# CUHK-AIM-Group/Depth-Aware-Endoscopy-SR

Hardware: AMD Instinct MI355X
Metric: LR frames/sec fwd+bwd at x8 (128x160 LR) (higher is better)
Workload: dtype f32; 1 GPU; Kvasir x8 synthetic, batch=16 per GPU, fp32, DepthNet nb=16 nf=64 L=256 K=10 (BASELINE.json configs[1]); step = fwd + L1 + dynamic loss + bwd + Adam; global_batch=16, scale=8, parallelism=dp1, mode=train, device=cuda, full=False, hip_graph=False

## Files before the change

depth-aware-endoscopy-sr_amd/csrc/edge.hip:

```cpp
#include "dasr_common.h"
#include "bf16.h"

extern "C" int dasr_version(void) { return 100; }
extern "C" int dasr_is_device_build(void) { return DASR_DEVICE_BUILD; }
extern "C" const char* dasr_error_string(int code) {
    switch (code) {
        case DASR_OK: return "ok";
        case DASR_E_NULL: return "null pointer argument";
        case DASR_E_SHAPE: return "inconsistent or non-positive sizes";
        case DASR_E_UNSUPPORTED: return "unsupported configuration";
        case DASR_E_WORKSPACE: return "workspace too small";
        default: return code > 0 ? "hip runtime error (hipError_t)" : "unknown error";
    }
}

__global__ void k_nchw_to_nhwc(const float* __restrict__ src, float* __restrict__ dst, int C, int HW, size_t n) {
    for (size_t i = (size_t)blockIdx.x * blockDim.x + threadIdx.x; i < n; i += (size_t)gridDim.x * blockDim.x) {
        size_t c = i % C, p = (i / C) % HW, b = i / ((size_t)C * HW);
        dst[i] = src[(b * C + c) * HW + p];
    }
}
__global__ void k_nhwc_to_nchw(const float* __restrict__ src, float* __restrict__ dst, int C, int HW, size_t n) {
    for (size_t i = (size_t)blockIdx.x * blockDim.x + threadIdx.x; i < n; i += (size_t)gridDim.x * blockDim.x) {
        size_t p = i % HW, c = (i / HW) % C, b = i / ((size_t)C * HW);
// ... 12 lines not shown
    DASR_CHECK_SHAPE(B > 0 && C > 0 && H > 0 && W > 0);
    size_t n = (size_t)B * C * H * W;
    DASR_LAUNCH(k_nhwc_to_nchw, dim3(dasr_ew_grid(n)), dim3(256), 0, stream, src, dst, C, H * W, n);
    DASR_RETURN_LAUNCH_STATUS();
}

__global__ void k_clamp_to_nchw(const float* __restrict__ y, float* __restrict__ out, int C, int HW, size_t n, float lo,
                                float hi) {
    for (size_t i = (size_t)blockIdx.x * blockDim.x + threadIdx.x; i < n; i += (size_t)gridDim.x * blockDim.x) {
        size_t p = i % HW, c = (i / HW) % C, b = i / ((size_t)C * HW);
        float v = y[(b * HW + p) * C + c];
        out[i] = fminf(fmaxf(v, lo), hi);
    }
}
__global__ void k_clamp_to_nchw_bwd(const float* __restrict__ dout, const float* __restrict__ y, float* __restrict__ dy,
                                    int C, int HW, size_t n, float lo, float hi) {
    for (size_t i = (size_t)blockIdx.x * blockDim.x + threadIdx.x; i < n; i += (size_t)gridDim.x * blockDim.x) {
        size_t c = i % C, p = (i / C) % HW, b = i / ((size_t)C * HW);
        float v = y[i];
        float g = dout[(b * C + c) * HW + p];
        dy[i] = (v >= lo && v <= hi) ? g : 0.f;
    }
}
extern "C" int dasr_clamp_to_nchw(const float* y, float* out, int B, int C, int H, int W, float lo, float hi,
                                  void* stream) {
    DASR_CHECK_PTR(y); DASR_CHECK_PTR(out);
    DASR_CHECK_SHAPE(B > 0 && C > 0 && H > 0 && W > 0);
    size_t n = (size_t)B * C * H * W;
    DASR_LAUNCH(k_clamp_to_nchw, dim3(dasr_ew_grid(n)), dim3(256), 0, stream, y, out, C, H * W, n, lo, hi);
    DASR_RETURN_LAUNCH_STATUS();
}
extern "C" int dasr_clamp_to_nchw_bwd(const float* dout, const float* y, float* dy, int B, int C, int H, int W, float lo,
                                      float hi, void* stream) {
    DASR_CHECK_PTR(dout); DASR_CHECK_PTR(y); DASR_CHECK_PTR(dy);
    DASR_CHECK_SHAPE(B > 0 && C > 0 && H > 0 && W > 0);
    size_t n = (size_t)B * C * H * W;
    DASR_LAUNCH(k_clamp_to_nchw_bwd, dim3(dasr_ew_grid(n)), dim3(256), 0, stream, dout, y, dy, C, H * W, n, lo, hi);
    DASR_RETURN_LAUNCH_STATUS();
}

__global__ void k_resize_nearest(const float* __restrict__ src, float* __restrict__ dst, int h, int w, int H, int W,
                                 size_t n) {
    float sh = (float)h / (float)H, sw = (float)w / (float)W;
    for (size_t i = (size_t)blockIdx.x * blockDim.x + threadIdx.x; i < n; i += (size_t)gridDim.x * blockDim.x) {
        int X = (int)(i % W), Y = (int)((i / W) % H);
        size_t bc = i / ((size_t)W * H);
        int y = (int)floorf((float)Y * sh); if (y > h - 1) y = h - 1;
        int x = (int)floorf((float)X * sw); if (x > w - 1) x = w - 1;
        dst[i] = src[(bc * h + y) * w + x];
    }
}
extern "C" int dasr_resize_nearest_nchw(const float* src, float* dst, int BC, int h, int w, int H, int W, void* stream) {
    DASR_CHECK_PTR(src); DASR_CHECK_PTR(dst);
    DASR_CHECK_SHAPE(BC > 0 && h > 0 && w > 0 && H > 0 && W > 0);
    size_t n = (size_t)BC * H * W;
    DASR_LAUNCH(k_resize_nearest, dim3(dasr_ew_grid(n)), dim3(256), 0, stream, src, dst, h, w, H, W, n);
    DASR_RETURN_LAUNCH_STATUS();
}

__global__ void k_resize_nearest_u8(const unsigned char* __restrict__ src, unsigned char* __restrict__ dst, int h, int w,
// ... 92 lines not shown
```

depth-aware-endoscopy-sr_amd/csrc/loss.hip:

```cpp
#include <stdint.h>

#include "dasr_common.h"

#define LOSS_MAXK 16

__global__ void __launch_bounds__(256) k_loss_sums(const float* __restrict__ sr, const float* __restrict__ hr,
                                                   const unsigned char* __restrict__ region, float* __restrict__ sums,
                                                   int B, int C, int h, int w, int s, int K) {
    __shared__ float red[2 * LOSS_MAXK + 2];
    for (int i = threadIdx.x; i < 2 * K + 1; i += 256) red[i] = 0.f;
    __syncthreads();
    const int W = w * s, H = h * s;
    const size_t nruns = (size_t)B * C * H * w;
    float l1 = 0.f;
    for (size_t r = (size_t)blockIdx.x * 256 + threadIdx.x; r < nruns; r += (size_t)gridDim.x * 256) {
        const int lx = (int)(r % w);
        const int Y = (int)((r / w) % H);
        const size_t bc = r / ((size_t)w * H);
        const int b = (int)(bc / C);
        const int k = region[((size_t)b * h + Y / s) * w + lx];
        const float* ps = sr + (bc * H + Y) * W + (size_t)lx * s;
        const float* ph = hr + (bc * H + Y) * W + (size_t)lx * s;
        float num = 0.f;
        for (int j = 0; j < s; ++j) {
            const float d = ps[j] - ph[j], ad = fabsf(d);
            l1 += ad;
            num += ad < 1.f ? 0.5f * d * d : ad - 0.5f;
        }
        if (k < K) {
            atomicAdd(&red[k], num);
            atomicAdd(&red[K + k], (float)s);
        }
    }
    for (int off = 32; off > 0; off >>= 1) l1 += __shfl_down(l1, off, 64);
    if ((threadIdx.x & 63) == 0) atomicAdd(&red[2 * K], l1);
    __syncthreads();
    for (int i = threadIdx.x; i < 2 * K + 1; i += 256) atomicAdd(&sums[i], red[i]);
}

__global__ void __launch_bounds__(256) k_loss_bwd(const float* __restrict__ sr, const float* __restrict__ hr,
                                                  const unsigned char* __restrict__ region,
                                                  const float* __restrict__ dsums, float* __restrict__ dsr, int B,
                                                  int C, int h, int w, int s, int K) {
    const int W = w * s, H = h * s;
    const size_t n = (size_t)B * C * H * W;
    const float dl1 = dsums[2 * K];
    for (size_t i = (size_t)blockIdx.x * 256 + threadIdx.x; i < n; i += (size_t)gridDim.x * 256) {
        const int X = (int)(i % W), Y = (int)((i / W) % H);
        const int b = (int)(i / ((size_t)W * H * C));
        const int k = region[((size_t)b * h + Y / s) * w + X / s];
        const float d = sr[i] - hr[i];
        const float sg = d > 0.f ? 1.f : (d < 0.f ? -1.f : 0.f);
        float g = dl1 * sg;
        if (k < K) g += dsums[k] * (fabsf(d) < 1.f ? d : sg);
        dsr[i] = g;
    }
}

extern "C" int dasr_loss_sums(const float* sr, const float* hr, const unsigned char* region, float* sums, int B, int C,
                              int h, int w, int scale, int K, void* stream) {
    DASR_CHECK_PTR(sr); DASR_CHECK_PTR(hr); DASR_CHECK_PTR(region); DASR_CHECK_PTR(sums);
    DASR_CHECK_SHAPE(B > 0 && C > 0 && h > 0 && w > 0 && scale > 0 && K > 0);
    if (K > LOSS_MAXK) return DASR_E_UNSUPPORTED;
    hipError_t e = hipMemsetAsync(sums, 0, sizeof(float) * (2 * K + 1), (hipStream_t)stream);
    if (e != hipSuccess) return (int)e;
    size_t nruns = (size_t)B * C * h * scale * w;
    DASR_LAUNCH(k_loss_sums, dim3(dasr_ew_grid(nruns)), dim3(256), 0, stream, sr, hr, region, sums, B, C, h, w, scale, K);
    DASR_RETURN_LAUNCH_STATUS();
}

extern "C" int dasr_loss_bwd(const float* sr, const float* hr, const unsigned char* region, const float* dsums,
                             float* dsr, int B, int C, int h, int w, int scale, int K, void* stream) {
    DASR_CHECK_PTR(sr); DASR_CHECK_PTR(hr); DASR_CHECK_PTR(region); DASR_CHECK_PTR(dsums); DASR_CHECK_PTR(dsr);
    DASR_CHECK_SHAPE(B > 0 && C > 0 && h > 0 && w > 0 && scale > 0 && K > 0);
    if (K > LOSS_MAXK) return DASR_E_UNSUPPORTED;
    size_t n = (size_t)B * C * h * scale * w * scale;
    DASR_LAUNCH(k_loss_bwd, dim3(dasr_ew_grid(n)), dim3(256), 0, stream, sr, hr, region, dsums, dsr, B, C, h, w, scale, K);
    DASR_RETURN_LAUNCH_STATUS();
}

__device__ __forceinline__ float loss_sign(float v) { return v > 0.f ? 1.f : (v < 0.f ? -1.f : 0.f); }

template <int K>
__device__ __forceinline__ void loss_soft_px(float d, const float (&m)[K], float (&num)[K], float& l1) {
    l1 += fabsf(d);
#pragma unroll
    for (int k = 0; k < K; ++k) {
        const float u = m[k] * d, au = fabsf(u);
        num[k] += au < 1.f ? 0.5f * u * u : au - 0.5f;
    }
// ... 89 lines not shown
    const float dl1 = dsums[2 * K];
    for (size_t r = (size_t)blockIdx.x * 256 + threadIdx.x; r < nruns; r += (size_t)gridDim.x * 256) {
        bool first_row;
        const size_t off = loss_soft_run<K>(r, mask, C, h, w, s, m, first_row);
#pragma unroll
        for (int k = 0; k < K; ++k) coef[k] = dnum[k] * m[k];
        for (int c = 0; c < C; ++c) {
            const float* ps = sr + off + c * plane;
            const float* ph = hr + off + c * plane;
            float* pd = dsr + off + c * plane;
            if (VEC) {
                for (int j = 0; j < s; j += 4) {
                    const f32x4 d = *reinterpret_cast<const f32x4*>(ps + j) - *reinterpret_cast<const f32x4*>(ph + j);
                    f32x4 g;
#pragma unroll
                    for (int i = 0; i < 4; ++i) g[i] = loss_soft_px_bwd<K>(d[i], dl1, m, coef);
                    *reinterpret_cast<f32x4*>(pd + j) = g;
                }
            } else {
                for (int j = 0; j < s; ++j) pd[j] = loss_soft_px_bwd<K>(ps[j] - ph[j], dl1, m, coef);
            }
        }
    }
}

static inline bool loss_aligned16(const void* a, const void* b, const void* c = nullptr) {
    return (((uintptr_t)a | (uintptr_t)b | (uintptr_t)c) & 15) == 0;
}

#define LOSS_SOFT_CASE(KK, KERNEL, ...)                                                                  \
    case KK:                                                                                             \
        if (vec) DASR_LAUNCH((KERNEL<KK, true>), dim3(dasr_ew_grid(nruns)), dim3(256), 0, stream, __VA_ARGS__);  \
        else DASR_LAUNCH((KERNEL<KK, false>), dim3(dasr_ew_grid(nruns)), dim3(256), 0, stream, __VA_ARGS__);     \
        break;
#define LOSS_SOFT_DISPATCH(KERNEL, ...)                                                                          \
    switch (K) {                                                                                                 \
        LOSS_SOFT_CASE(1, KERNEL, __VA_ARGS__) LOSS_SOFT_CASE(2, KERNEL, __VA_ARGS__) LOSS_SOFT_CASE(3, KERNEL, __VA_ARGS__)    \
        LOSS_SOFT_CASE(4, KERNEL, __VA_ARGS__) LOSS_SOFT_CASE(5, KERNEL, __VA_ARGS__) LOSS_SOFT_CASE(6, KERNEL, __VA_ARGS__)    \
        LOSS_SOFT_CASE(7, KERNEL, __VA_ARGS__) LOSS_SOFT_CASE(8, KERNEL, __VA_ARGS__) LOSS_SOFT_CASE(9, KERNEL, __VA_ARGS__)    \
        LOSS_SOFT_CASE(10, KERNEL, __VA_ARGS__) LOSS_SOFT_CASE(11, KERNEL, __VA_ARGS__) LOSS_SOFT_CASE(12, KERNEL, __VA_ARGS__) \
        LOSS_SOFT_CASE(13, KERNEL, __VA_ARGS__) LOSS_SOFT_CASE(14, KERNEL, __VA_ARGS__) LOSS_SOFT_CASE(15, KERNEL, __VA_ARGS__) \
        LOSS_SOFT_CASE(16, KERNEL, __VA_ARGS__)                                                                  \
        default: return DASR_E_UNSUPPORTED;                                                                      \
    }

extern "C" int dasr_loss_sums_soft(const float* sr, const float* hr, const float* mask, float* sums, int B, int C, int h,
                                   int w, int scale, int K, void* stream) {
    DASR_CHECK_PTR(sr); DASR_CHECK_PTR(hr); DASR_CHECK_PTR(mask); DASR_CHECK_PTR(sums);
    DASR_CHECK_SHAPE(B > 0 && C > 0 && h > 0 && w > 0 && scale > 0 && K > 0);
    if (K > LOSS_MAXK) return DASR_E_UNSUPPORTED;
// ... 316 lines not shown
```

depth-aware-endoscopy-sr_amd/depthnet.py:

```python
import contextlib
import math

import torch
import torch.nn as nn

from . import graph
from .tape import Tape, Var


def _default_conv_init_(weight, bias, fan_in):
    bound = 1.0 / math.sqrt(fan_in)
    with torch.no_grad():
        weight.uniform_(-bound, bound)
        if bias is not None:
            bias.uniform_(-bound, bound)


class _PlainConv(nn.Module):

    def __init__(self, cin, cout, k):
        super().__init__()
        self.cin, self.cout, self.k = cin, cout, k
        self.weight = nn.Parameter(torch.empty(cout, cin, k, k))
        self.bias = nn.Parameter(torch.empty(cout))
# ... 64 lines not shown

    forward = _PlainConv.forward


class _Encoder(nn.Module):

    def __init__(self, in_nc, latent):
        super().__init__()
        self.layer1 = _WNConv(in_nc, 32)
        self.layer2 = _WNConv(32, 64)
        self.layer3 = _WNConv(64, 128)
        self.layer4 = _WNConv(128, latent, transposed=True)
        self.layer5 = _WNConv(latent, latent)

    forward = _PlainConv.forward


def _device_guard(t):
    return torch.cuda.device(t.device) if t.is_cuda else contextlib.nullcontext()


class _DepthNetFunction(torch.autograd.Function):
    @staticmethod
    def forward(ctx, net, act_dtype, inp, depth_map, depth_mask, region, *params):
        tape = Tape(enabled=True, act_dtype=act_dtype)
        tape.prepack = net._prepack_for(inp.device, act_dtype)
        pvars = [Var(p.detach(), p.requires_grad, name) for name, p in zip(net._param_names, params)]
        P = {v.name: v for v in pvars}
        out = graph.depthnet_forward(tape, P, net.cfg, net._consts(inp.device), inp.detach().contiguous(),
                                     depth_map.detach().contiguous(), depth_mask.detach().contiguous(), region)
        ctx.tape, ctx.pvars, ctx.out = tape, pvars, out
        ctx.hook = getattr(net, "_grad_bucket_hook", None)
        return out.data

    @staticmethod
    def backward(ctx, dout):
        tape, pvars, out = ctx.tape, ctx.pvars, ctx.out
        if tape is None:
            raise RuntimeError("DepthNet: backward called twice on the same forward")
        out.grad = dout.contiguous()
        if ctx.hook is not None:
            hook = ctx.hook
            tape.on_mark = lambda: hook(pvars)
        with _device_guard(dout):
            tape.backward()
        grads = tuple(v.grad for v in pvars)
        for v in pvars:
            v.grad = None
        ctx.tape = ctx.pvars = ctx.out = ctx.hook = None
        return (None, None, None, None, None, None) + grads


class DepthNet(nn.Module):
    def __init__(self, which_ResBlk_depth=[], in_nc=3, out_nc=3, nf=64, nb=16, scale=4, input_para=10, min=0.0,
                 max=1.0, depth_latent_ch=256, depthRangeNum=10, norm_type='weight_norm', use_trainable_params=True,
                 norm_gamma=0.1, norm_beta=0.1, ablate_depth_matrix=False, ablate_depth_block=False):
        super().__init__()
        if norm_type != 'weight_norm':
            raise NotImplementedError("dasr_amd.DepthNet: only norm_type='weight_norm' (all shipped ymls) is built")
        if ablate_depth_matrix or ablate_depth_block:
            raise NotImplementedError("dasr_amd.DepthNet: the ablate_* variants are outside the hot path (SURVEY §8b)")
        if scale not in (2, 3, 4, 8):
            raise NotImplementedError("dasr_amd.DepthNet: scale must be 2, 3, 4 or 8")
        self.scale, self.min, self.max, self.para = scale, min, max, input_para
        self.num_blocks = nb
        self.which_ResBlk_depth = list(which_ResBlk_depth)
        self.isBaseline = len(self.which_ResBlk_depth) == 0
        self.ablate_depth_matrix, self.ablate_depth_block = False, False
        self.cfg = dict(which_ResBlk_depth=self.which_ResBlk_depth, in_nc=in_nc, out_nc=out_nc, nf=nf, nb=nb,
                        scale=scale, depth_latent_ch=depth_latent_ch, depthRangeNum=depthRangeNum,
                        use_trainable_params=use_trainable_params, norm_gamma=norm_gamma, norm_beta=norm_beta,
                        out_min=float(min), out_max=float(max))

# ... 80 lines not shown
            P = {name: Var(p.detach(), False, name) for name, p in zip(self._param_names, params)}
            return graph.depthnet_infer_nhwc(tape, P, self.cfg, self._consts(x_nhwc.device), x_nhwc, depthMap, depthMask,
                                             graph.attached_region(depthMask))

    def forward(self, input, depthMap, depthMask):
        with _device_guard(input):
            return self._forward(input, depthMap, depthMask)

    def _forward(self, input, depthMap, depthMask):
        params = self._resolve_params()
        for t, nm in ((depthMap, "depthMap"), (depthMask, "depthMask")):
            if t.device != input.device:
                raise ValueError("DepthNet: %s is on %s, input on %s" % (nm, t.device, input.device))
        if params and params[0].device != input.device:
            raise ValueError("DepthNet: parameters on %s, input on %s" % (params[0].device, input.device))
        for t, nm in ((input, "input"), (depthMap, "depthMap"), (depthMask, "depthMask")):
            if t.dtype != torch.float32:
                raise TypeError("DepthNet: %s must be float32" % nm)
        if input.dim() != 4 or depthMap.dim() != 4 or depthMask.dim() != 4:
            raise ValueError("DepthNet: expected 4-D NCHW tensors")
        region = graph.attached_region(depthMask)
        act_dtype = self._act_dtype(input.device)
        if torch.is_grad_enabled() and any(p.requires_grad for p in params):
            return _DepthNetFunction.apply(self, act_dtype, input, depthMap, depthMask, region, *params)
        tape = Tape(enabled=False, act_dtype=act_dtype)
        if not self.training:
            if not hasattr(self, "_fold_cache"):
                object.__setattr__(self, "_fold_cache", {})
            tape.fold_cache = self._fold_cache
        P = {name: Var(p.detach(), False, name) for name, p in zip(self._param_names, params)}
        out = graph.depthnet_forward(tape, P, self.cfg, self._consts(input.device), input.detach().contiguous(),
                                     depthMap.detach().contiguous(), depthMask.detach().contiguous(), region)
        return out.data
```

depth-aware-endoscopy-sr_amd/graph.py:

```python
import math

import torch

from . import ops
from .tape import Tape, Var, accum


FUSE_DGRAD_ACT = False
FUSE_C9_DGRAD_ACT = True
FUSE_SPLIT_DGRAD_ACT = True

SIDE_STREAM = True
import os as _os
import threading as _threading
TAIL_WGRAD_SIDE = False
FUSE_INSTNORM_STATS = False
ENCODER_S2D = True
SPLIT_BF16 = True
SPLIT_WGRAD = True
SPLIT_PIECES = 2
FUSE_AMAX = True
SPLIT_CONV9 = True
SPLIT_MIN_PIXELS = 1 << 14
WGRAD_STREAM = False
_SIDE = {}
_SIDE_LOCK = _threading.Lock()


def _side_stream(device, which="branch"):
    key = (str(device), which)
    with _SIDE_LOCK:
        if key not in _SIDE:
            _SIDE[key] = torch.cuda.Stream(device=device, priority=-1)
# ... 720 lines not shown
    s2d_ok = all(P["encoder.layer%d.weight_v" % i].data.shape[0] % 32 == 0 and
                 P["encoder.layer%d.weight_v" % i].data.shape[1] % 32 == 0 for i in (2, 3, 4, 5))
    if len(cfg["which_ResBlk_depth"]) > 0 and tape.act_dtype == torch.bfloat16 and ENCODER_S2D and s2d_ok:
        def s2(name, x, act, valid_hw=None):
            return conv(tape, space_to_depth2(tape, x, valid_hw), expand_s2(tape, _wn(tape, P, name)), P[name + ".bias"],
                        act=act)
        e2 = s2("encoder.layer2", e1, L)
        e3 = s2("encoder.layer3", e2, L)
        w4, b4 = expand_t2(tape, _wn(tape, P, "encoder.layer4", True), P["encoder.layer4.bias"])
        e4 = conv(tape, e3, w4, b4, act=L, ps_r=2)
        H3, W3 = e3.data.shape[1], e3.data.shape[2]
        e5 = to_f32(tape, s2("encoder.layer5", e4, ops.ACT_NONE, (2 * H3 - 1, 2 * W3 - 1)))
        st = region_pool(tape, e5, depth_mask)
    elif len(cfg["which_ResBlk_depth"]) > 0:
        e2 = conv(tape, e1, _wn(tape, P, "encoder.layer2"), P["encoder.layer2.bias"], stride=2, act=L)
        e3 = conv(tape, e2, _wn(tape, P, "encoder.layer3"), P["encoder.layer3.bias"], stride=2, act=L)
        e4 = conv(tape, e3, _wn(tape, P, "encoder.layer4", True), P["encoder.layer4.bias"], stride=2,
                  transposed=True, act=L)
        e5 = conv(tape, e4, _wn(tape, P, "encoder.layer5"), P["encoder.layer5.bias"], stride=2)
        st = region_pool(tape, e5, depth_mask)
    return e1, e5, st


def depthnet_forward(tape, P, cfg, consts, inp, depth_map, depth_mask, region=None):
    pp = tape.prepack
    if pp is not None and not (PREPACK and tape.enabled and pp.lock.acquire(blocking=False)):
        pp = tape.prepack = None
    try:
        if pp is not None:
            pp.begin(P, Prepack.signature(inp, tape.act_dtype))
        out = _depthnet_forward(tape, P, cfg, consts, inp, depth_map, depth_mask, region)
        if pp is not None:
            pp.finish()
        return out
    finally:
        if pp is not None:
            pp.lock.release()


def depthnet_infer_nhwc(tape, P, cfg, consts, x_nhwc, depth_map, depth_mask, region=None):
    if tape.enabled:
        raise ValueError("depthnet_infer_nhwc is an inference entry: the tape must be off")
    return _depthnet_forward(tape, P, cfg, consts, x_nhwc, depth_map, depth_mask, region, nhwc=True).data


def _depthnet_forward(tape, P, cfg, consts, inp, depth_map, depth_mask, region, *, nhwc=False):
    plan = block_plan(cfg)
    nb, scale = cfg["nb"], cfg["scale"]
    B = inp.shape[0]
    x0 = Var(inp if nhwc else ops.nchw_to_nhwc(inp))
    dm = Var(depth_map.reshape(B, depth_map.shape[2], depth_map.shape[3], 1))
    L = ops.ACT_LRELU
    e1, _e5, st = encoder_forward(tape, P, cfg, x0, depth_mask)
    mask_pack = MaskPack(depth_mask, region) if st is not None else None
    adt = tape.act_dtype
    e1h = to_bf16(tape, e1) if adt == torch.bfloat16 else e1
    h1 = conv(tape, e1h, _wn(tape, P, "head.0", dtype=adt), P["head.0.bias"], act=L)
    fea_bef = conv(tape, h1, _wn(tape, P, "head.2", dtype=adt), P["head.2.bias"], act=L)

    executed = list(range(nb - 3)) + [nb - 2, nb - 1]
    branch = {}
    side = _side_stream(inp.device) if (SIDE_STREAM and inp.is_cuda and mask_pack is not None) else None
    if side is not None:
        main = torch.cuda.current_stream()
        side.wait_stream(main)
        feat_hw = {}
        hw = (x0.data.shape[1], x0.data.shape[2])
        for i in executed:
            if i == nb - 2 and scale == 8:
# ... 15 lines not shown
                branch[i] = tuple(pair)

    def run_block(i, x):
        name, kind, _ = plan[i]
        if kind == "depth":
            return depth_block(tape, P, name, x, dm, mask_pack, st, consts, branch.get(i))
        return classic_block(tape, P, name, x)

    fea = fea_bef
    tape.mark()
    for i in range(nb - 3):
        fea = run_block(i, fea)
        if i == (nb - 3) // 2 - 1:
            tape.mark()
    fea = add(tape, fea, fea_bef)
    tape.mark()
    if scale == 8:
        fea = upscale(tape, P, "upscale1", fea, 2, True)
    fea = run_block(nb - 2, fea)
    if scale >= 4:
        fea = upscale(tape, P, "upscale2", fea, 2, True)
    fea = run_block(nb - 1, fea)
    fea = upscale(tape, P, "upscale3", fea, 3 if scale == 3 else 2, False)
    y = conv(tape, fea, pack(tape, P["conv_output.weight"]), P["conv_output.bias"], pad=4, side_wgrad=True)
    if nhwc:
        return y
    lo, hi = cfg["out_min"], cfg["out_max"]
    out = Var(ops.clamp_to_nchw(y.data, lo, hi), True)

    def bwd():
        if out.grad is None:
            return
        accum(y, ops.clamp_to_nchw_bwd(out.grad, y.data, lo, hi))
        out.grad = None

    tape.record(bwd)
    return out
```

depth-aware-endoscopy-sr_amd/harness.py:

```python
import math

import torch
import torch.nn.functional as F


def cosine_restart_lr(step, base_lr=1e-3, T_period=(20000, 20000, 20000, 20000),
                      restarts=(20000, 40000, 60000), weights=(1, 1, 1), eta_min=1e-7):
    last_restart, T, w = 0, T_period[0], 1.0
    for j, r in enumerate(restarts):
        if step >= r:
            last_restart, T, w = r, T_period[j + 1], weights[j]
    return eta_min + (base_lr * w - eta_min) * (1 + math.cos(math.pi * (step - last_restart) / T)) / 2


def _world(group=None):
    if torch.distributed.is_available() and torch.distributed.is_initialized():
        return torch.distributed.get_world_size(group)
    return 1


class _RegionSums(torch.autograd.Function):

    @staticmethod
    def forward(ctx, sr, hr, region, K):
        from . import ops
        sr_c, hr_c = sr.contiguous(), hr.contiguous()
        ctx.save_for_backward(sr_c, hr_c, region)
        ctx.K = K
        return ops.loss_sums(sr_c, hr_c, region, K)

    @staticmethod
    def backward(ctx, dsums):
        from . import ops
        sr, hr, region = ctx.saved_tensors
        return ops.loss_bwd(sr, hr, region, dsums.contiguous(), ctx.K), None, None, None


class _RegionSumsSoft(torch.autograd.Function):

    @staticmethod
    def forward(ctx, sr, hr, mask, K):
        from . import ops
        sr_c, hr_c, mask_c = sr.contiguous(), hr.contiguous(), mask.detach().contiguous()
        ctx.save_for_backward(sr_c, hr_c, mask_c)
        ctx.K = K
        return ops.loss_sums_soft(sr_c, hr_c, mask_c, K)

    @staticmethod
    def backward(ctx, dsums):
        from . import ops
        sr, hr, mask = ctx.saved_tensors
        return ops.loss_bwd_soft(sr, hr, mask, dsums.contiguous(), ctx.K), None, None, None


def ssim_torch(img1, img2):
    from .validate import _window_1d
    g = _window_1d().unsqueeze(1)
# ... 601 lines not shown
```

depth-aware-endoscopy-sr_amd/ops.py:

```python
import ctypes

import torch

from . import _lib

ACT_NONE, ACT_RELU, ACT_LRELU = 0, 1, 2
IN_EPS = 1e-5


BF16 = torch.bfloat16


def _p(t, allow_none=False):
    return _lib.ptr(t, allow_none)


def _pa(t, allow_none=False):
    if t is None:
        return _lib.ptr(t, allow_none)
    return _lib.ptr(t, allow_none, dtype=t.dtype if t.dtype in (torch.float32, BF16) else torch.float32)


def _is_bf(*ts):
    kinds = {t.dtype for t in ts if t is not None}
# ... 740 lines not shown
    dfeat = torch.empty(feat_shape, dtype=torch.float32, device=dout.device)
    _call("dasr_region_pool_bwd", _p(dout), _p(maskr), _p(area), _p(dfeat), B, K, L, h, w)
    return dfeat


def loss_sums(sr, hr, region, K):
    B, C, H, W = sr.shape
    _, h, w = region.shape
    scale = H // h
    assert H == h * scale and W == w * scale
    sums = empty((2 * K + 1,), sr)
    _call("dasr_loss_sums", _p(sr), _p(hr), _lib.ptr(region, dtype=torch.uint8), _p(sums), B, C, h, w, scale, K)
    return sums


def loss_bwd(sr, hr, region, dsums, K):
    B, C, H, W = sr.shape
    _, h, w = region.shape
    dsr = torch.empty_like(sr)
    _call("dasr_loss_bwd", _p(sr), _p(hr), _lib.ptr(region, dtype=torch.uint8), _p(dsums), _p(dsr), B, C, h, w, H // h, K)
    return dsr


LOSS_MAX_REGIONS = 16


def _soft_loss_dims(sr, mask, K):
    B, C, H, W = sr.shape
    Bm, Km, h, w = mask.shape
    scale = H // h
    assert (Bm, Km) == (B, K) and H == h * scale and W == w * scale
    return B, C, h, w, scale


def loss_sums_soft(sr, hr, mask, K):
    B, C, h, w, scale = _soft_loss_dims(sr, mask, K)
    assert hr.shape == sr.shape
    sums = empty((2 * K + 1,), sr)
    _call("dasr_loss_sums_soft", _p(sr), _p(hr), _p(mask), _p(sums), B, C, h, w, scale, K)
    return sums


def loss_bwd_soft(sr, hr, mask, dsums, K):
    B, C, h, w, scale = _soft_loss_dims(sr, mask, K)
    assert hr.shape == sr.shape and dsums.numel() == 2 * K + 1
    dsr = torch.empty_like(sr)
# ... 197 lines not shown
```

include/dasr.h:

```cpp
#ifndef DASR_H
#define DASR_H

#include <stddef.h>
#include <stdint.h>

#ifdef __cplusplus
extern "C" {
#endif

#define DASR_OK 0
#define DASR_E_NULL (-1)
#define DASR_E_SHAPE (-2)
#define DASR_E_UNSUPPORTED (-3)
#define DASR_E_WORKSPACE (-4)

#define DASR_ACT_NONE 0
#define DASR_ACT_RELU 1
#define DASR_ACT_LRELU02 2

int dasr_version(void);
const char* dasr_error_string(int code);
int dasr_is_device_build(void);

int dasr_nchw_to_nhwc(const float* src, float* dst, int B, int C, int H, int W, void* stream);
// ... 117 lines not shown
                  float* dbias_gamma, float* dbias_beta, float* dalpha_gamma, float* dalpha_beta, float* dres,
                  float* dt_amax, float* dgb2_amax, void* workspace, size_t workspace_bytes, int relu, int B, int H, int W,
                  int C, int K, float eps, void* stream);

int dasr_sean_soft_mask_max_regions(void);

int dasr_region_pool_fwd(const float* feat, const float* mask, float* maskr, float* area, float* out, int B, int K,
                         int L, int h, int w, int H, int W, void* stream);
int dasr_region_pool_bwd(const float* dout, const float* maskr, const float* area, float* dfeat, int B, int K, int L,
                         int h, int w, void* stream);

size_t dasr_depth_to_masks_workspace(int B, int HW);
int dasr_depth_to_masks(const float* depth, const float* fixed_edges, float* masks, unsigned char* region,
                        void* workspace, size_t workspace_bytes, int B, int HW, int K, void* stream);

size_t dasr_depth_to_masks_soft_workspace(int B, int HW);
int dasr_depth_to_masks_soft(const float* depth, float* masks, void* workspace, size_t workspace_bytes, int B, int HW,
                             int K, float width, int fixed_range, void* stream);

int dasr_loss_sums(const float* sr, const float* hr, const unsigned char* region, float* sums, int B, int C, int h,
                   int w, int scale, int K, void* stream);
int dasr_loss_bwd(const float* sr, const float* hr, const unsigned char* region, const float* dsums, float* dsr, int B,
                  int C, int h, int w, int scale, int K, void* stream);
int dasr_loss_sums_soft(const float* sr, const float* hr, const float* mask, float* sums, int B, int C, int h, int w,
                        int scale, int K, void* stream);
int dasr_loss_bwd_soft(const float* sr, const float* hr, const float* mask, const float* dsums, float* dsr, int B, int C,
                       int h, int w, int scale, int K, void* stream);
#define DASR_CRIT_NONE (-1)
#define DASR_CRIT_L1 0
#define DASR_CRIT_L2 1
#define DASR_CRIT_CB 2
#define DASR_CRIT_SMOOTHL1 3
int dasr_loss_sums_crit(const float* sr, const float* hr, const unsigned char* region, float* sums, int B, int C, int h,
                        int w, int scale, int K, int pixel_crit, int crit_a, int crit_b, void* stream);
int dasr_loss_bwd_crit(const float* sr, const float* hr, const unsigned char* region, const float* dsums, float* dsr,
                       int B, int C, int h, int w, int scale, int K, int pixel_crit, int crit_a, int crit_b, void* stream);
int dasr_loss_sums_soft_crit(const float* sr, const float* hr, const float* mask, float* sums, int B, int C, int h, int w,
                             int scale, int K, int pixel_crit, int crit_a, int crit_b, void* stream);
int dasr_loss_bwd_soft_crit(const float* sr, const float* hr, const float* mask, const float* dsums, float* dsr, int B,
                            int C, int h, int w, int scale, int K, int pixel_crit, int crit_a, int crit_b, void* stream);

int dasr_add(const float* a, const float* b, float* out, size_t n, void* stream);
int dasr_accumulate(float* dst, const float* src, size_t n, void* stream);
int dasr_copy(float* dst, const float* src, size_t n, void* stream);


// ... 79 lines not shown
```

Measured before the change: 263.3 frames/s.

## Fuse loss backward with clamp/NCHW backward and vectorize loss and clamp kernels

Adds a loss handle that lets the dynamic loss backward write the gradient directly in NHWC w.r.t. the pre-clamp conv output. This fuses the loss gradient, the clamp mask and the layout transpose into one kernel, which can also emit the amax, and a zero-stride placeholder is passed back through autograd so the separate clamp backward is skipped. It also adds float4-vectorized per-batch kernels for the loss sums, using per-thread region accumulators instead of shared atomics, and for the clamp transpose forward and backward. The cost is coupling between the loss function and the network autograd through a side-channel handle, plus template instantiation over K.

```diff
diff --git a/depth-aware-endoscopy-sr_amd/csrc/edge.hip b/depth-aware-endoscopy-sr_amd/csrc/edge.hip
--- a/depth-aware-endoscopy-sr_amd/csrc/edge.hip
+++ b/depth-aware-endoscopy-sr_amd/csrc/edge.hip
@@ -1,3 +1,5 @@
+#include <stdint.h>
+
 #include "dasr_common.h"
 #include "bf16.h"
 
@@ -58,12 +60,74 @@
         dy[i] = (v >= lo && v <= hi) ? g : 0.f;
     }
 }
+__global__ void __launch_bounds__(256) k_clamp_to_nchw_v4(const float* __restrict__ y, float* __restrict__ out,
+                                                          unsigned HW, float lo, float hi) {
+    const float* yb = y + (size_t)blockIdx.y * HW * 3;
+    float* ob = out + (size_t)blockIdx.y * HW * 3;
+    const unsigned n4 = HW >> 2;
+    for (unsigned q = blockIdx.x * 256 + threadIdx.x; q < n4; q += gridDim.x * 256) {
+        float v[12];
+#pragma unroll
+        for (int j = 0; j < 3; ++j) {
+            const f32x4 t = *reinterpret_cast<const f32x4*>(yb + 12 * q + 4 * j);
+            v[4 * j] = t[0]; v[4 * j + 1] = t[1]; v[4 * j + 2] = t[2]; v[4 * j + 3] = t[3];
+        }
+#pragma unroll
+        for (int c = 0; c < 3; ++c) {
+            f32x4 o;
+#pragma unroll
+            for (int i = 0; i < 4; ++i) o[i] = fminf(fmaxf(v[3 * i + c], lo), hi);
+            *reinterpret_cast<f32x4*>(ob + c * HW + 4 * q) = o;
+        }
+    }
+}
+__global__ void __launch_bounds__(256) k_clamp_to_nchw_bwd_v4(const float* __restrict__ dout, const float* __restrict__ y,
+                                                              float* __restrict__ dy, unsigned HW, float lo, float hi) {
+    const float* yb = y + (size_t)blockIdx.y * HW * 3;
+    const float* gb = dout + (size_t)blockIdx.y * HW * 3;
+    float* db = dy + (size_t)blockIdx.y * HW * 3;
+    const unsigned n4 = HW >> 2;
+    for (unsigned q = blockIdx.x * 256 + threadIdx.x; q < n4; q += gridDim.x * 256) {
+        float v[12], g[12];
+#pragma unroll
+        for (int j = 0; j < 3; ++j) {
+            const f32x4 t = *reinterpret_cast<const f32x4*>(yb + 12 * q + 4 * j);
+            v[4 * j] = t[0]; v[4 * j + 1] = t[1]; v[4 * j + 2] = t[2]; v[4 * j + 3] = t[3];
+        }
+#pragma unroll
+        for (int c = 0; c < 3; ++c) {
+            const f32x4 t = *reinterpret_cast<const f32x4*>(gb + c * HW + 4 * q);
+#pragma unroll
+            for (int i = 0; i < 4; ++i) g[3 * i + c] = t[i];
+        }
+#pragma unroll
+        for (int j = 0; j < 3; ++j) {
+            f32x4 o;
+#pragma unroll
+            for (int i = 0; i < 4; ++i) o[i] = (v[4 * j + i] >= lo && v[4 * j + i] <= hi) ? g[4 * j + i] : 0.f;
+            *reinterpret_cast<f32x4*>(db + 12 * q + 4 * j) = o;
+        }
+    }
+}
+static inline bool edge_v4_ok(int B, int C, int H, int W, const void* a, const void* b, const void* c = nullptr) {
+    const size_t HW = (size_t)H * W;
+    return C == 3 && HW % 4 == 0 && 3 * HW < ((size_t)1 << 31) && B <= 65535 &&
+           (((uintptr_t)a | (uintptr_t)b | (uintptr_t)c) & 15) == 0;
+}
+static inline unsigned edge_v4_gx(int B, size_t HW) {
+    unsigned gx = dasr_cdiv(HW / 4, 256), cap = 2048u / (unsigned)B;
+    if (cap < 1) cap = 1;
+    return gx < cap ? gx : cap;
+}
 extern "C" int dasr_clamp_to_nchw(const float* y, float* out, int B, int C, int H, int W, float lo, float hi,
                                   void* stream) {
     DASR_CHECK_PTR(y); DASR_CHECK_PTR(out);
     DASR_CHECK_SHAPE(B > 0 && C > 0 && H > 0 && W > 0);
     size_t n = (size_t)B * C * H * W;
-    DASR_LAUNCH(k_clamp_to_nchw, dim3(dasr_ew_grid(n)), dim3(256), 0, stream, y, out, C, H * W, n, lo, hi);
+    if (edge_v4_ok(B, C, H, W, y, out))
+        DASR_LAUNCH(k_clamp_to_nchw_v4, dim3(edge_v4_gx(B, (size_t)H * W), B), dim3(256), 0, stream, y, out, (unsigned)(H * W), lo, hi);
+    else
+        DASR_LAUNCH(k_clamp_to_nchw, dim3(dasr_ew_grid(n)), dim3(256), 0, stream, y, out, C, H * W, n, lo, hi);
     DASR_RETURN_LAUNCH_STATUS();
 }
 extern "C" int dasr_clamp_to_nchw_bwd(const float* dout, const float* y, float* dy, int B, int C, int H, int W, float lo,
@@ -71,7 +135,10 @@
     DASR_CHECK_PTR(dout); DASR_CHECK_PTR(y); DASR_CHECK_PTR(dy);
     DASR_CHECK_SHAPE(B > 0 && C > 0 && H > 0 && W > 0);
     size_t n = (size_t)B * C * H * W;
-    DASR_LAUNCH(k_clamp_to_nchw_bwd, dim3(dasr_ew_grid(n)), dim3(256), 0, stream, dout, y, dy, C, H * W, n, lo, hi);
+    if (edge_v4_ok(B, C, H, W, dout, y, dy))
+        DASR_LAUNCH(k_clamp_to_nchw_bwd_v4, dim3(edge_v4_gx(B, (size_t)H * W), B), dim3(256), 0, stream, dout, y, dy, (unsigned)(H * W), lo, hi);
+    else
+        DASR_LAUNCH(k_clamp_to_nchw_bwd, dim3(dasr_ew_grid(n)), dim3(256), 0, stream, dout, y, dy, C, H * W, n, lo, hi);
     DASR_RETURN_LAUNCH_STATUS();
 }
 
diff --git a/depth-aware-endoscopy-sr_amd/csrc/loss.hip b/depth-aware-endoscopy-sr_amd/csrc/loss.hip
--- a/depth-aware-endoscopy-sr_amd/csrc/loss.hip
+++ b/depth-aware-endoscopy-sr_amd/csrc/loss.hip
@@ -38,6 +38,72 @@
     for (int i = threadIdx.x; i < 2 * K + 1; i += 256) atomicAdd(&sums[i], red[i]);
 }
 
+template <int K>
+__global__ void __launch_bounds__(256) k_loss_sums_v4(const float* __restrict__ sr, const float* __restrict__ hr,
+                                                      const unsigned char* __restrict__ region, float* __restrict__ sums,
+                                                      int C, int h, int w, int s) {
+    __shared__ float red[2 * LOSS_MAXK + 1];
+    for (int i = threadIdx.x; i < 2 * K + 1; i += 256) red[i] = 0.f;
+    __syncthreads();
+    const unsigned W = (unsigned)w * s, H = (unsigned)h * s;
+    const size_t plane = (size_t)H * W;
+    const float* srb = sr + (size_t)blockIdx.y * C * plane;
+    const float* hrb = hr + (size_t)blockIdx.y * C * plane;
+    const unsigned char* rb = region + (size_t)blockIdx.y * h * w;
+    const unsigned nruns = H * (unsigned)w;
+    float num[K], cnt[K], l1 = 0.f;
+#pragma unroll
+    for (int k = 0; k < K; ++k) num[k] = cnt[k] = 0.f;
+    for (unsigned r = blockIdx.x * 256 + threadIdx.x; r < nruns; r += gridDim.x * 256) {
+        const unsigned Y = r / (unsigned)w, lx = r - Y * (unsigned)w;
+        const int kr = rb[(Y / (unsigned)s) * (unsigned)w + lx];
+        const unsigned off = Y * W + lx * (unsigned)s;
+        float run = 0.f;
+        for (int c = 0; c < C; ++c) {
+            const float* ps = srb + c * plane + off;
+            const float* ph = hrb + c * plane + off;
+            for (int j = 0; j < s; j += 4) {
+                const f32x4 d4 = *reinterpret_cast<const f32x4*>(ps + j) - *reinterpret_cast<const f32x4*>(ph + j);
+#pragma unroll
+                for (int i = 0; i < 4; ++i) {
+                    const float d = d4[i], ad = fabsf(d);
+                    l1 += ad;
+                    run += ad < 1.f ? 0.5f * d * d : ad - 0.5f;
+                }
+            }
+        }
+#pragma unroll
+        for (int k = 0; k < K; ++k) {
+            num[k] += kr == k ? run : 0.f;
+            cnt[k] += kr == k ? 1.f : 0.f;
+        }
+    }
+    const float area_scale = (float)C * (float)s;
+#pragma unroll
+    for (int k = 0; k < K; ++k) {
+        float a = num[k], b = cnt[k];
+        for (int off = 32; off > 0; off >>= 1) {
+            a += __shfl_down(a, off, 64);
+            b += __shfl_down(b, off, 64);
+        }
+        if ((threadIdx.x & 63) == 0) {
+            atomicAdd(&red[k], a);
+            atomicAdd(&red[K + k], b * area_scale);
+        }
+    }
+    for (int off = 32; off > 0; off >>= 1) l1 += __shfl_down(l1, off, 64);
+    if ((threadIdx.x & 63) == 0) atomicAdd(&red[2 * K], l1);
+    __syncthreads();
+    for (int i = threadIdx.x; i < 2 * K + 1; i += 256) atomicAdd(&sums[i], red[i]);
+}
+
+__device__ __forceinline__ float loss_onehot_grad(float d, float dl1, bool has, float dk) {
+    const float sg = d > 0.f ? 1.f : (d < 0.f ? -1.f : 0.f);
+    float g = dl1 * sg;
+    if (has) g += dk * (fabsf(d) < 1.f ? d : sg);
+    return g;
+}
+
 __global__ void __launch_bounds__(256) k_loss_bwd(const float* __restrict__ sr, const float* __restrict__ hr,
                                                   const unsigned char* __restrict__ region,
                                                   const float* __restrict__ dsums, float* __restrict__ dsr, int B,
@@ -49,12 +115,102 @@
         const int X = (int)(i % W), Y = (int)((i / W) % H);
         const int b = (int)(i / ((size_t)W * H * C));
         const int k = region[((size_t)b * h + Y / s) * w + X / s];
-        const float d = sr[i] - hr[i];
-        const float sg = d > 0.f ? 1.f : (d < 0.f ? -1.f : 0.f);
-        float g = dl1 * sg;
-        if (k < K) g += dsums[k] * (fabsf(d) < 1.f ? d : sg);
-        dsr[i] = g;
-    }
+        dsr[i] = loss_onehot_grad(sr[i] - hr[i], dl1, k < K, k < K ? dsums[k] : 0.f);
+    }
+}
+
+__global__ void __launch_bounds__(256) k_loss_bwd_nhwc(const float* __restrict__ y, const float* __restrict__ hr,
+                                                       const unsigned char* __restrict__ region,
+                                                       const float* __restrict__ dsums, float* __restrict__ dy,
+                                                       float* __restrict__ amax, int B, int C, int h, int w, int s, int K,
+                                                       float lo, float hi) {
+    __shared__ float s_part[16];
+    const int W = w * s, H = h * s;
+    const size_t HW = (size_t)H * W, n = (size_t)B * C * HW;
+    const float dl1 = dsums[2 * K];
+    float m = 0.f;
+    for (size_t i = (size_t)blockIdx.x * 256 + threadIdx.x; i < n; i += (size_t)gridDim.x * 256) {
+        const size_t c = i % C, p = (i / C) % HW, b = i / ((size_t)C * HW);
+        const int X = (int)(p % W), Y = (int)(p / W);
+        const int k = region[(b * h + Y / s) * w + X / s];
+        const float v = y[i];
+        const float d = fminf(fmaxf(v, lo), hi) - hr[(b * C + c) * HW + p];
+        const float g = loss_onehot_grad(d, dl1, k < K, k < K ? dsums[k] : 0.f);
+        const float o = (v >= lo && v <= hi) ? g : 0.f;
+        dy[i] = o;
+        m = dasr_amax1(m, o);
+    }
+    if (amax) dasr_amax_commit(amax, m, s_part, dasr_flat_wg(), dasr_flat_nwg());
+}
+
+template <bool ONE_REGION>
+__global__ void __launch_bounds__(256) k_loss_bwd_nhwc_v4(const float* __restrict__ y, const float* __restrict__ hr,
+                                                          const unsigned char* __restrict__ region,
+                                                          const float* __restrict__ dsums, float* __restrict__ dy,
+                                                          float* __restrict__ amax, int h, int w, int s, int K, float lo,
+                                                          float hi) {
+    __shared__ float s_part[16];
+    const unsigned W = (unsigned)w * s, HW = (unsigned)h * s * W, n4 = HW >> 2;
+    const float* yb = y + (size_t)blockIdx.y * HW * 3;
+    const float* hb = hr + (size_t)blockIdx.y * HW * 3;
+    float* db = dy + (size_t)blockIdx.y * HW * 3;
+    const unsigned char* rb = region + (size_t)blockIdx.y * h * w;
+    const float dl1 = dsums[2 * K];
+    float m = 0.f;
+    for (unsigned q = blockIdx.x * 256 + threadIdx.x; q < n4; q += gridDim.x * 256) {
+        bool has[4];
+        float dk[4];
+        if (ONE_REGION) {
+            const unsigned Y = (4 * q) / W, X = 4 * q - Y * W;
+            const int k = rb[(Y / (unsigned)s) * (unsigned)w + X / (unsigned)s];
+            const float t = k < K ? dsums[k] : 0.f;
+#pragma unroll
+            for (int i = 0; i < 4; ++i) { has[i] = k < K; dk[i] = t; }
+        } else {
+#pragma unroll
+            for (int i = 0; i < 4; ++i) {
+                const unsigned Y = (4 * q + i) / W, X = 4 * q + i - Y * W;
+                const int k = rb[(Y / (unsigned)s) * (unsigned)w + X / (unsigned)s];
+                has[i] = k < K;
+                dk[i] = k < K ? dsums[k] : 0.f;
+            }
+        }
+        float v[12], t[12];
+#pragma unroll
+        for (int j = 0; j < 3; ++j) {
+            const f32x4 a = *reinterpret_cast<const f32x4*>(yb + 12 * q + 4 * j);
+            v[4 * j] = a[0]; v[4 * j + 1] = a[1]; v[4 * j + 2] = a[2]; v[4 * j + 3] = a[3];
+        }
+#pragma unroll
+        for (int c = 0; c < 3; ++c) {
+            const f32x4 a = *reinterpret_cast<const f32x4*>(hb + c * HW + 4 * q);
+#pragma unroll
+            for (int i = 0; i < 4; ++i) t[3 * i + c] = a[i];
+        }
+#pragma unroll
+        for (int j = 0; j < 3; ++j) {
+            f32x4 o;
+#pragma unroll
+            for (int i = 0; i < 4; ++i) {
+                const int e = 4 * j + i;
+                const float d = fminf(fmaxf(v[e], lo), hi) - t[e];
+                const float g = loss_onehot_grad(d, dl1, has[e / 3], dk[e / 3]);
+                o[i] = (v[e] >= lo && v[e] <= hi) ? g : 0.f;
+                m = dasr_amax1(m, o[i]);
+            }
+            *reinterpret_cast<f32x4*>(db + 12 * q + 4 * j) = o;
+        }
+    }
+    if (amax) dasr_amax_commit(amax, m, s_part, dasr_flat_wg(), dasr_flat_nwg());
+}
+
+static inline bool loss_aligned16(const void* a, const void* b, const void* c = nullptr) {
+    return (((uintptr_t)a | (uintptr_t)b | (uintptr_t)c) & 15) == 0;
+}
+static inline unsigned loss_gx(int B, size_t n) {
+    unsigned gx = dasr_cdiv(n, 256), cap = 2048u / (unsigned)B;
+    if (cap < 1) cap = 1;
+    return gx < cap ? gx : cap;
 }
 
 extern "C" int dasr_loss_sums(const float* sr, const float* hr, const unsigned char* region, float* sums, int B, int C,
@@ -65,7 +221,40 @@
     hipError_t e = hipMemsetAsync(sums, 0, sizeof(float) * (2 * K + 1), (hipStream_t)stream);
     if (e != hipSuccess) return (int)e;
     size_t nruns = (size_t)B * C * h * scale * w;
+    const size_t plane = (size_t)h * scale * w * scale;
+    if (scale % 4 == 0 && loss_aligned16(sr, hr) && plane < ((size_t)1 << 31) && B <= 65535) {
+        const dim3 grid(loss_gx(B, (size_t)h * scale * w), B);
+        switch (K) {
+#define LOSS_V4_CASE(KK) case KK: DASR_LAUNCH((k_loss_sums_v4<KK>), grid, dim3(256), 0, stream, sr, hr, region, sums, C, h, w, scale); break;
+            LOSS_V4_CASE(1) LOSS_V4_CASE(2) LOSS_V4_CASE(3) LOSS_V4_CASE(4) LOSS_V4_CASE(5) LOSS_V4_CASE(6) LOSS_V4_CASE(7)
+            LOSS_V4_CASE(8) LOSS_V4_CASE(9) LOSS_V4_CASE(10) LOSS_V4_CASE(11) LOSS_V4_CASE(12) LOSS_V4_CASE(13)
+            LOSS_V4_CASE(14) LOSS_V4_CASE(15) LOSS_V4_CASE(16)
+#undef LOSS_V4_CASE
+            default: return DASR_E_UNSUPPORTED;
+        }
+        DASR_RETURN_LAUNCH_STATUS();
+    }
     DASR_LAUNCH(k_loss_sums, dim3(dasr_ew_grid(nruns)), dim3(256), 0, stream, sr, hr, region, sums, B, C, h, w, scale, K);
+    DASR_RETURN_LAUNCH_STATUS();
+}
+
+extern "C" int dasr_loss_bwd_nhwc(const float* y, const float* hr, const unsigned char* region, const float* dsums,
+                                  float* dy, float* dy_amax, int B, int C, int h, int w, int scale, int K, float lo,
+                                  float hi, void* stream) {
+    DASR_CHECK_PTR(y); DASR_CHECK_PTR(hr); DASR_CHECK_PTR(region); DASR_CHECK_PTR(dsums); DASR_CHECK_PTR(dy);
+    DASR_CHECK_SHAPE(B > 0 && C > 0 && h > 0 && w > 0 && scale > 0 && K > 0);
+    if (K > LOSS_MAXK) return DASR_E_UNSUPPORTED;
+    const size_t HW = (size_t)h * scale * w * scale;
+    if (C == 3 && HW % 4 == 0 && 3 * HW < ((size_t)1 << 31) && B <= DASR_AMAX_MAX_PARTS && loss_aligned16(y, hr, dy)) {
+        const dim3 grid(loss_gx(B, HW / 4), B);
+        if (scale % 4 == 0)
+            DASR_LAUNCH((k_loss_bwd_nhwc_v4<true>), grid, dim3(256), 0, stream, y, hr, region, dsums, dy, dy_amax, h, w, scale, K, lo, hi);
+        else
+            DASR_LAUNCH((k_loss_bwd_nhwc_v4<false>), grid, dim3(256), 0, stream, y, hr, region, dsums, dy, dy_amax, h, w, scale, K, lo, hi);
+        DASR_RETURN_LAUNCH_STATUS();
+    }
+    DASR_LAUNCH(k_loss_bwd_nhwc, dim3(dasr_ew_grid(C * B * HW)), dim3(256), 0, stream, y, hr, region, dsums, dy, dy_amax, B, C, h,
+                w, scale, K, lo, hi);
     DASR_RETURN_LAUNCH_STATUS();
 }
 
@@ -201,10 +390,6 @@
             }
         }
     }
-}
-
-static inline bool loss_aligned16(const void* a, const void* b, const void* c = nullptr) {
-    return (((uintptr_t)a | (uintptr_t)b | (uintptr_t)c) & 15) == 0;
 }
 
 #define LOSS_SOFT_CASE(KK, KERNEL, ...)                                                                  \
diff --git a/depth-aware-endoscopy-sr_amd/depthnet.py b/depth-aware-endoscopy-sr_amd/depthnet.py
--- a/depth-aware-endoscopy-sr_amd/depthnet.py
+++ b/depth-aware-endoscopy-sr_amd/depthnet.py
@@ -110,14 +110,15 @@
 
 class _DepthNetFunction(torch.autograd.Function):
     @staticmethod
-    def forward(ctx, net, act_dtype, inp, depth_map, depth_mask, region, *params):
+    def forward(ctx, net, act_dtype, hand, inp, depth_map, depth_mask, region, *params):
         tape = Tape(enabled=True, act_dtype=act_dtype)
         tape.prepack = net._prepack_for(inp.device, act_dtype)
         pvars = [Var(p.detach(), p.requires_grad, name) for name, p in zip(net._param_names, params)]
         P = {v.name: v for v in pvars}
         out = graph.depthnet_forward(tape, P, net.cfg, net._consts(inp.device), inp.detach().contiguous(),
-                                     depth_map.detach().contiguous(), depth_mask.detach().contiguous(), region)
-        ctx.tape, ctx.pvars, ctx.out = tape, pvars, out
+                                     depth_map.detach().contiguous(), depth_mask.detach().contiguous(), region,
+                                     loss_handle=hand)
+        ctx.tape, ctx.pvars, ctx.out, ctx.hand = tape, pvars, out, hand
         ctx.hook = getattr(net, "_grad_bucket_hook", None)
         return out.data
 
@@ -126,7 +127,7 @@
         tape, pvars, out = ctx.tape, ctx.pvars, ctx.out
         if tape is None:
             raise RuntimeError("DepthNet: backward called twice on the same forward")
-        out.grad = dout.contiguous()
+        out.grad = None if (ctx.hand is not None and ctx.hand.is_placeholder(dout)) else dout.contiguous()
         if ctx.hook is not None:
             hook = ctx.hook
             tape.on_mark = lambda: hook(pvars)
@@ -135,8 +136,8 @@
         grads = tuple(v.grad for v in pvars)
         for v in pvars:
             v.grad = None
-        ctx.tape = ctx.pvars = ctx.out = ctx.hook = None
-        return (None, None, None, None, None, None) + grads
+        ctx.tape = ctx.pvars = ctx.out = ctx.hook = ctx.hand = None
+        return (None, None, None, None, None, None, None) + grads
 
 
 class DepthNet(nn.Module):
@@ -263,7 +264,11 @@
         region = graph.attached_region(depthMask)
         act_dtype = self._act_dtype(input.device)
         if torch.is_grad_enabled() and any(p.requires_grad for p in params):
-            return _DepthNetFunction.apply(self, act_dtype, input, depthMap, depthMask, region, *params)
+            hand = graph.LossHandle() if graph.FUSE_LOSS_BWD else None
+            sr = _DepthNetFunction.apply(self, act_dtype, hand, input, depthMap, depthMask, region, *params)
+            if hand is not None and hand.y is not None:
+                sr._dasr_loss_handle = hand
+            return sr
         tape = Tape(enabled=False, act_dtype=act_dtype)
         if not self.training:
             if not hasattr(self, "_fold_cache"):
diff --git a/depth-aware-endoscopy-sr_amd/graph.py b/depth-aware-endoscopy-sr_amd/graph.py
--- a/depth-aware-endoscopy-sr_amd/graph.py
+++ b/depth-aware-endoscopy-sr_amd/graph.py
@@ -9,6 +9,7 @@
 FUSE_DGRAD_ACT = False
 FUSE_C9_DGRAD_ACT = True
 FUSE_SPLIT_DGRAD_ACT = True
+FUSE_LOSS_BWD = True
 
 SIDE_STREAM = True
 import os as _os
@@ -775,14 +776,14 @@
     return e1, e5, st
 
 
-def depthnet_forward(tape, P, cfg, consts, inp, depth_map, depth_mask, region=None):
+def depthnet_forward(tape, P, cfg, consts, inp, depth_map, depth_mask, region=None, loss_handle=None):
     pp = tape.prepack
     if pp is not None and not (PREPACK and tape.enabled and pp.lock.acquire(blocking=False)):
         pp = tape.prepack = None
     try:
         if pp is not None:
             pp.begin(P, Prepack.signature(inp, tape.act_dtype))
-        out = _depthnet_forward(tape, P, cfg, consts, inp, depth_map, depth_mask, region)
+        out = _depthnet_forward(tape, P, cfg, consts, inp, depth_map, depth_mask, region, loss_handle=loss_handle)
         if pp is not None:
             pp.finish()
         return out
@@ -797,7 +798,7 @@
     return _depthnet_forward(tape, P, cfg, consts, x_nhwc, depth_map, depth_mask, region, nhwc=True).data
 
 
-def _depthnet_forward(tape, P, cfg, consts, inp, depth_map, depth_mask, region, *, nhwc=False):
+def _depthnet_forward(tape, P, cfg, consts, inp, depth_map, depth_mask, region, *, nhwc=False, loss_handle=None):
     plan = block_plan(cfg)
     nb, scale = cfg["nb"], cfg["scale"]
     B = inp.shape[0]
@@ -859,17 +860,61 @@
         fea = upscale(tape, P, "upscale2", fea, 2, True)
     fea = run_block(nb - 1, fea)
     fea = upscale(tape, P, "upscale3", fea, 3 if scale == 3 else 2, False)
-    y = conv(tape, fea, pack(tape, P["conv_output.weight"]), P["conv_output.bias"], pad=4, side_wgrad=True)
+    return output_tail(tape, P, cfg, fea, nhwc=nhwc, loss_handle=loss_handle)
+
+
+def output_tail(tape, P, cfg, fea, *, nhwc=False, loss_handle=None):
+    w9 = pack(tape, P["conv_output.weight"])
+    y = conv(tape, fea, w9, P["conv_output.bias"], pad=4, side_wgrad=True)
     if nhwc:
         return y
     lo, hi = cfg["out_min"], cfg["out_max"]
     out = Var(ops.clamp_to_nchw(y.data, lo, hi), True)
-
-    def bwd():
-        if out.grad is None:
-            return
-        accum(y, ops.clamp_to_nchw_bwd(out.grad, y.data, lo, hi))
-        out.grad = None
-
-    tape.record(bwd)
-    return out
+    hand = loss_handle if (FUSE_LOSS_BWD and tape.enabled and y.data.dtype == torch.float32) else None
+    if hand is not None:
+        hand.offer(y.data, lo, hi, want_amax=FUSE_AMAX and _is_c9(w9))
+
+    def bwd():
+        dy = hand.take() if hand is not None else None
+        if dy is not None:
+            accum(y, dy)
+        if out.grad is not None:
+            accum(y, ops.clamp_to_nchw_bwd(out.grad, y.data, lo, hi))
+            out.grad = None
+
+    tape.record(bwd)
+    return out
+
+
+class LossHandle:
+    __slots__ = ("y", "lo", "hi", "dy", "want_amax", "zero")
+    _ZERO = {}
+
+    def __init__(self):
+        self.y = self.dy = self.zero = None
+        self.lo = self.hi = 0.0
+        self.want_amax = False
+
+    def offer(self, y, lo, hi, want_amax):
+        self.y, self.lo, self.hi, self.want_amax = y, lo, hi, want_amax
+        key = str(y.device)
+        if key not in LossHandle._ZERO:
+            LossHandle._ZERO[key] = torch.zeros((), dtype=torch.float32, device=y.device)
+        self.zero = LossHandle._ZERO[key]
+
+    def open(self):
+        return self.y is not None and self.dy is None
+
+    def placeholder(self, shape):
+        return self.zero.expand(shape)
+
+    def is_placeholder(self, dout):
+        return (self.dy is not None and dout.data_ptr() == self.zero.data_ptr() and all(s == 0 for s in dout.stride()))
+
+    def take(self):
+        dy, self.dy, self.y = self.dy, None, None
+        return dy
+
+
+def loss_handle_of(sr):
+    return getattr(sr, "_dasr_loss_handle", None) if FUSE_LOSS_BWD else None
diff --git a/depth-aware-endoscopy-sr_amd/harness.py b/depth-aware-endoscopy-sr_amd/harness.py
--- a/depth-aware-endoscopy-sr_amd/harness.py
+++ b/depth-aware-endoscopy-sr_amd/harness.py
@@ -23,16 +23,22 @@
 
     @staticmethod
     def forward(ctx, sr, hr, region, K):
-        from . import ops
+        from . import graph, ops
         sr_c, hr_c = sr.contiguous(), hr.contiguous()
         ctx.save_for_backward(sr_c, hr_c, region)
         ctx.K = K
+        ctx.hand = graph.loss_handle_of(sr) if sr_c is sr else None
         return ops.loss_sums(sr_c, hr_c, region, K)
 
     @staticmethod
     def backward(ctx, dsums):
         from . import ops
         sr, hr, region = ctx.saved_tensors
+        hand = ctx.hand
+        if hand is not None and hand.open() and hand.y.device == hr.device:
+            amax = ops.amax_buffer(hand.y) if hand.want_amax else None
+            hand.dy = ops.loss_bwd_nhwc(hand.y, hr, region, dsums.contiguous(), ctx.K, hand.lo, hand.hi, amax=amax)
+            return hand.placeholder(sr.shape), None, None, None
         return ops.loss_bwd(sr, hr, region, dsums.contiguous(), ctx.K), None, None, None
 
 
diff --git a/depth-aware-endoscopy-sr_amd/ops.py b/depth-aware-endoscopy-sr_amd/ops.py
--- a/depth-aware-endoscopy-sr_amd/ops.py
+++ b/depth-aware-endoscopy-sr_amd/ops.py
@@ -786,6 +786,17 @@
     return dsr
 
 
+def loss_bwd_nhwc(y, hr, region, dsums, K, lo, hi, amax=None):
+    B, H, W, C = y.shape
+    _, h, w = region.shape
+    scale = H // h
+    assert tuple(hr.shape) == (B, C, H, W) and H == h * scale and W == w * scale and dsums.numel() == 2 * K + 1
+    dy = empty(y.shape, y)
+    _call("dasr_loss_bwd_nhwc", _p(y), _p(hr), _lib.ptr(region, dtype=torch.uint8), _p(dsums), _p(dy), _p(amax, True), B, C,
+          h, w, scale, K, float(lo), float(hi))
+    return set_amax(dy, amax)
+
+
 LOSS_MAX_REGIONS = 16
 
 
diff --git a/include/dasr.h b/include/dasr.h
--- a/include/dasr.h
+++ b/include/dasr.h
@@ -163,6 +163,9 @@
                    int w, int scale, int K, void* stream);
 int dasr_loss_bwd(const float* sr, const float* hr, const unsigned char* region, const float* dsums, float* dsr, int B,
                   int C, int h, int w, int scale, int K, void* stream);
+int dasr_loss_bwd_nhwc(const float* y_nhwc, const float* hr, const unsigned char* region, const float* dsums,
+                       float* dy_nhwc, float* dy_amax, int B, int C, int h, int w, int scale, int K, float lo, float hi,
+                       void* stream);
 int dasr_loss_sums_soft(const float* sr, const float* hr, const float* mask, float* sums, int B, int C, int h, int w,
                         int scale, int K, void* stream);
 int dasr_loss_bwd_soft(const float* sr, const float* hr, const float* mask, const float* dsums, float* dsr, int B, int C,
```

New measurement: 266.0 frames/s, median of 6. +1.0%, better.
